# xyang9527/dro-sfm

Measured on AMD Instinct MI355X. Metric: training images/sec (KITTI 192x640 mf self-sup), higher is better.
Workload: dtype f32; 1 GPU; KITTI 192x640 mf self-sup (configs[1]); model=DepthPoseNet it8-seq4-inter-out, global_batch=2, per_gpu_batch=2, ref_frames=2, parallelism=dp1, optimizer=Adam lr 2e-4, execution=hipgraph, update_blocks=depth block + pose block (side stream, with both context encoders), encoder_3x3_s1=hip, encoder_strided=hip, exchange=none (world 1)

## Files before the change

### dro-sfm_amd/csrc/conv.hip

```cpp
#include <hip/hip_runtime.h>

#include <algorithm>
#include <climits>
#include <cstddef>
#include <cstdio>
#include <cstdlib>
#include <cstring>
#include <map>
#include <mutex>
#include <string>
#include <type_traits>

#include "conv_common.hpp"
#include "dro_common.hpp"
#include "wgrad_group_plan.hpp"

namespace dro {


template <int BM, int MODE, int ACT, int EPI>
__global__ __launch_bounds__(256) void igemm_kernel(IgArgs a) {
  constexpr int WM = BM / 32;
  constexpr int KSTEPS = (WM == 2) ? 16 : 8;
  __shared__ float Ws[2][kBK][BM + 1];
// ... 295 lines not shown
}

template <int BM, int KH, int KW, int MODE, int ACT, int EPI, int KS, int XF = 0>
__global__ __launch_bounds__(256 * KS) void dconv_kernel(IgArgs a) {
  using S = HaloShape<BM, KH, KW>;
  {
    const unsigned long long t0 = __builtin_amdgcn_s_memtime();
    if (a.stamps && (threadIdx.x == 0 || threadIdx.x == blockDim.x - 64))
      a.stamps[(size_t)blockIdx.x * 16 + (threadIdx.x == 0 ? 10 : 11)] = t0;
  }
  constexpr int PF = KS <= 2 ? 2 : 1;
  static_assert(KS == 1 || S::LDS >= 4 * 16 * 64, "cross-group reduction area");
  constexpr int T = S::T, TH = S::TH, TW = S::TW, HWd = S::HWd, HALO = S::HALO, HPAD = S::HPAD;
  constexpr int CK = S::CK, NJ = S::NJ, XPER = CK / 4;
  constexpr int RUN = MODE == 0 ? S::RUN0 : S::RUN1, WS = MODE == 0 ? S::WS0 : S::WS1;
  constexpr int WSZ = MODE == 0 ? S::WSZ0 : S::WSZ1, STAGE = S::STAGE;
  constexpr int WM = BM / 32;
  constexpr int PH = KH / 2, PW = KW / 2;
  __shared__ float smem_all[KS * S::LDS];
  const int cb1 = a.cbase[1], cb2 = a.cbase[2], cb3 = a.cbase[3];
  const int H = a.g.H, W = a.g.W;
  const int Cin = a.g.Cin, Cout = a.g.Cout, rows = a.rows, kch = a.kch;
  const int CinT = (MODE == 1 ? a.wcin : Cin) * T;
  const float* __restrict__ Wt = a.weight;
  const float* __restrict__ Gp = a.G;
  const int tid = threadIdx.x & 255, lane = tid & 63;
  const int grp = KS == 1 ? 0 : __builtin_amdgcn_readfirstlane(threadIdx.x >> 8);
  const int wave = __builtin_amdgcn_readfirstlane(tid >> 6);
  float* smem = smem_all + grp * S::LDS;
  const int tile = xcd_remap(blockIdx.x, gridDim.x);
  const int pt = (int)udiv((unsigned)tile, a.rt_div), rt = tile - pt * a.row_tiles;
  const int row0 = rt * BM;
  if constexpr (MODE == 1 && XF == 0 && EPI < 5) {
    const int rl = min(row0 + BM, rows) - 1;
    const int s0 = (row0 >= cb1) + (row0 >= cb2) + (row0 >= cb3);
    const int s1 = (rl >= cb1) + (rl >= cb2) + (rl >= cb3);
    const float* t0 = s0 == 0 ? a.gsrc[0] : s0 == 1 ? a.gsrc[1] : s0 == 2 ? a.gsrc[2] : a.gsrc[3];
    if (s0 == s1 && t0 == nullptr) return;
  }
  const int wcol0 = MODE == 1 ? row0 + (row0 >= a.wgap_at ? a.wgap_len : 0) : row0;
  const int b = (int)udiv((unsigned)pt, a.ti_div), trem = pt - b * a.tiles_img;
  const int tyi = (int)udiv((unsigned)trem, a.tx_div);
  const int ty0 = tyi * TH, tx0 = (trem - tyi * a.tiles_x) * TW;
  const size_t HW = (size_t)H * W;
  const unsigned HWu = (unsigned)HW;
  const int nck = (kch + CK - 1) / CK;
  const int cbeg = blockIdx.y * a.chunks_per_split;
  const int cend = min(nck, cbeg + a.chunks_per_split);

  unsigned xpb[NJ];
  bool xok[NJ], own[NJ];
  static_assert(XF == 0 || ((MODE == 0) == (XF != 3) && ACT == 0), "BN staging transforms: XF 1/2 forward, 3 data gradient");
#pragma unroll
  for (int j = 0; j < NJ; ++j) {
    const int e = lane + 64 * j;
    const int hy = e / HWd, hx = e - hy * HWd;
    const int yy = ty0 - PH + hy, xx = tx0 - PW + hx;
    xok[j] = e < HALO && (unsigned)yy < (unsigned)H && (unsigned)xx < (unsigned)W;
    xpb[j] = xok[j] ? 4u * (unsigned)(yy * W + xx) : 0u;
    own[j] = XF != 0 && xok[j] && hy >= PH && hy < PH + TH && hx >= PW && hx < PW + TW;
  }
  const unsigned wlast = (unsigned)Cout * CinT - 1;

  unsigned long long sQ[4];
  unsigned sR[4], sM[4];
#pragma unroll
  for (int t = 0; t < 4; ++t) {
    if (MODE == 0) {
      sQ[t] = a.sq0[t] + (unsigned long long)b * a.sqb[t];
      sR[t] = a.sr[t];
      sM[t] = a.sm[t];
    } else {
      sQ[t] = reinterpret_cast<unsigned long long>(Gp) + 4ull * (unsigned long long)b * Cout * HW;
      sR[t] = 4u * HWu;
      sM[t] = ~0u;
    }
  }
  const unsigned long long dQ1 = sQ[1] - sQ[0], dQ2 = sQ[2] - sQ[1], dQ3 = sQ[3] - sQ[2];
  const unsigned dR1 = sR[1] - sR[0], dR2 = sR[2] - sR[1], dR3 = sR[3] - sR[2];
  const unsigned dM1 = sM[1] - sM[0], dM2 = sM[2] - sM[1], dM3 = sM[3] - sM[2];
  const long long sbase = MODE == 0 ? reinterpret_cast<long long>(a.src[0].p) : reinterpret_cast<long long>(Gp);
  const long long yshift = reinterpret_cast<long long>(XF == 2 ? a.bn.skip : XF == 3 ? a.bn.z : a.gy) - sbase;
  const long long oshift = reinterpret_cast<long long>(a.bn.yout) - sbase;

  constexpr bool FOLD = MODE == 1 && ACT != 0;
  constexpr bool Y2 = FOLD || XF == 2 || XF == 3;
  constexpr int NXC = XF == 3 ? 5 : 3;
  const float galpha = a.galpha;
  constexpr int W4 = S::WTOT / 4, WPER4 = (W4 + 255) / 256;
  constexpr int WREG = 4 * WPER4;
  static_assert(S::WTOT % 4 == 0 && RUN % 4 == 0, "float4 weight runs");
  unsigned woff[WPER4];
  int wdst[WPER4];
#pragma unroll
  for (int i = 0; i < WPER4; ++i) {
    const int e = 4 * (tid + 256 * i);
    const int run = e / RUN, rem = e - run * RUN;
    woff[i] = (unsigned)run * CinT + (unsigned)rem;
    wdst[i] = (W4 % 256 == 0 || e < S::WTOT) ? run * WS + rem : -1;
  }
  typedef __attribute__((address_space(1))) char* GWPtr;
  struct Stage {
    float xr[XPER * NJ], yr[Y2 ? XPER * NJ : 1], wv[WREG];
    unsigned cmask;
    unsigned ownc;
// ... 274 lines not shown
    }
    if (rowt && !(a.bn.dbg & 2)) bn_put(a.bn.part + (size_t)pt * rows + row, s1, s2);
    if (a.bn.inkernel) bn_finish<EPI>(a, pt, rt, row0, BM);
    stamp(14);
    return;
  }
  for (int e = threadIdx.x; e < BM * 64; e += 256 * KS) {
    const int rl = e >> 6, pl = e & 63;
    float v = 0.f;
#pragma unroll
    for (int g = 0; g < KS; ++g) {
      if (WM == 1)
        v += smem_all[((size_t)(2 * g) * BM + rl) * 64 + pl] + smem_all[((size_t)(2 * g + 1) * BM + rl) * 64 + pl];
      else
        v += smem_all[((size_t)g * BM + rl) * 64 + pl];
    }
    const int row = row0 + rl;
    const int py = pl / TW, px = pl - py * TW;
    const int oy = ty0 + py, ox = tx0 + px;
    if (row >= rows || oy >= H || ox >= W) continue;
    const size_t epix = (size_t)oy * W + ox;
    if (a.part)
      a.part[(size_t)blockIdx.y * rows * P + (size_t)row * P + (size_t)b * HW + epix] = v;
    else
      epi_store<MODE, ACT, EPI>(a, row, b, epix, HW, v);
  }
  stamp(14);
}


__global__ __launch_bounds__(256) void wgrad_kernel(IgArgs a) {
  constexpr int NB = 1;
  __shared__ float Gs[NB][kWP][64 + 1];
  __shared__ float Xs[NB][kWP][64 + 1];
  const int cb1 = a.cbase[1], cb2 = a.cbase[2], cb3 = a.cbase[3];
  const int H = a.g.H, W = a.g.W, KW = a.g.KW, PH = a.g.PH, PW = a.g.PW;
  const int Hsrc = a.Hs, Wsrc = a.Ws, sh = a.sshift;
  const unsigned HWs = (unsigned)Hsrc * (unsigned)Wsrc;
  const int Cin = a.g.Cin, Cout = a.g.Cout;
  const float* __restrict__ Gp = a.G;
  const FastDiv cindiv = a.cindiv, kwdiv = a.kwdiv;
  const int tid = threadIdx.x, lane = tid & 63, wave = tid >> 6;
  const int t = blockIdx.x;
  const int ot = t % a.otiles, nt = t / a.otiles;
  const int o0 = ot * 64, n0 = nt * 64;
  const int NK = a.K;
// ... 1387 lines not shown
      set_error("conv2d: BatchNorm fusion needs a 3x3 stride-1 halo convolution");
      return DRO_E_SHAPE;
    }
    if (EPI >= 5) {
      pl.chunks_per_split = (a.kch + pl.CK - 1) / pl.CK;
      pl.ksplit = 1;
    }
  }
  a.stamps = g_conv_stamps;
  a.dbg = 0;
  if (g_conv_stamps) {
    const char* e = getenv("DRO_CONV_DBG");
    a.dbg = e ? atoi(e) : 0;
  }
  a.K = a.kch * a.g.KH * a.g.KW;
  static const bool thin_off = getenv("DRO_CONV_NO_THIN") != nullptr;
  if (!BNF && !a.flat_only && !thin_off && thin_ok<MODE, EPI>(a)) {
    a.part = reinterpret_cast<float*>(ws);
    return launch_thin<MODE, ACT>(a, pl.ksplit, s);
  }
  if constexpr (EPI < 3 && !BNF) {
    if (!a.flat_only && a.wsplit && xconv_supported(a.g.KH, a.g.KW)) return launch_xconv<MODE, ACT, EPI>(a, ws, s);
  }
  a.row_tiles = pl.row_tiles;
  a.chunks_per_split = pl.chunks_per_split;
  a.part = pl.ksplit > 1 ? reinterpret_cast<float*>(ws) : nullptr;
  const dim3 grid(pl.row_tiles * pl.ptiles, pl.ksplit);
  const double flops = 2.0 * a.rows * a.kch * a.g.KH * a.g.KW * (double)P;
  if (pl.halo)
    conv_logf(flops, "dconv_kernel<%d, %d, %d, %d, %d, %d, %d>", pl.bm, a.g.KH, a.g.KW, MODE, ACT, EPI, pl.kin);
  else
    conv_logf(flops, "igemm_kernel<%d, %d, %d, %d>", pl.bm, MODE, ACT, EPI);
  if (pl.halo) {
    a.TH = pl.TH;
    a.TW = pl.TW;
    a.HWd = pl.HWd;
    a.HPAD = pl.HPAD;
    a.tiles_x = pl.tiles_x;
    a.tiles_img = pl.tiles_img;
    a.CK = pl.CK;
    a.rt_div = make_div32(pl.row_tiles);
    a.ti_div = make_div32(pl.tiles_img);
    a.tx_div = make_div32(pl.tiles_x);
    if (MODE == 0) {
      const unsigned long long HWl = (unsigned long long)a.g.H * a.g.W;
      for (int t = 0; t < kMaxSrc; ++t) {
        const Slice& sl = a.src[t];
        const unsigned long long chs = sl.bcast ? 1ull : HWl;
        const long long cbt = t == 0 ? 0 : a.cbase[t];
        a.sq0[t] = reinterpret_cast<unsigned long long>(sl.p) +
                   4ull * (unsigned long long)(((long long)sl.coff - cbt) * (long long)chs);
        a.sqb[t] = 4ull * (unsigned long long)sl.ctot * chs;
        a.sr[t] = 4u * (unsigned)chs;
        a.sm[t] = sl.bcast ? 0u : ~0u;
      }
    }
    const int KH = a.g.KH;
    const int KW = a.g.KW;
#define DRO_DCONV(BM_, KH_, KW_)                                                                    \
    do {                                                                                            \
      if (pl.kin == 4)                                                                              \
        hipLaunchKernelGGL((dconv_kernel<BM_, KH_, KW_, MODE, ACT, EPI, 4, XF>), grid, dim3(1024), 0, s, a); \
      else if (pl.kin == 2)                                                                         \
        hipLaunchKernelGGL((dconv_kernel<BM_, KH_, KW_, MODE, ACT, EPI, 2, XF>), grid, dim3(512), 0, s, a);  \
// ... 684 lines not shown

extern "C" int dro_conv2d_backward(const dro_slice* srcs, int nsrc, const float* weight, int B, int H,
                                   int W, int Cout, int KH, int KW, int act, float alpha,
                                   const dro_slice* y, const float* dout, float* const* grad_srcs,
                                   const int* grad_ctot, const int* grad_coff,
                                   const int* grad_accumulate, float* grad_weight, float* grad_bias,
                                   int grad_weight_accumulate, const void* wsplit, void* workspace,
                                   size_t workspace_bytes, void* stream) {
  return conv2d_backward_impl(srcs, nsrc, weight, B, H, W, Cout, KH, KW, act, alpha, y, dout, grad_srcs,
                              grad_ctot, grad_coff, grad_accumulate, grad_weight, grad_bias,
                              grad_weight_accumulate, wsplit, workspace, workspace_bytes, stream, nullptr);
}

extern "C" int dro_conv2d_backward_gapped(const dro_slice* srcs, int nsrc, const float* weight, int wcin,
                                          int gap_at, int gap_len, int B, int H, int W, int Cout, int KH,
                                          int KW, const float* dout, float* const* grad_srcs,
                                          const int* grad_ctot, const int* grad_coff,
                                          const int* grad_accumulate, void* workspace, size_t workspace_bytes,
                                          void* stream) {
  const WeightGap gap = {wcin, gap_at, gap_len};
  return conv2d_backward_impl(srcs, nsrc, weight, B, H, W, Cout, KH, KW, 0, 1.f, nullptr, dout, grad_srcs,
                              grad_ctot, grad_coff, grad_accumulate, nullptr, nullptr, 0, nullptr, workspace,
                              workspace_bytes, stream, nullptr, &gap);
}

extern "C" int dro_convgru_candidate_backward(const dro_slice* srcs, int nsrc, const float* weight, int B,
                                              int H, int W, int hd, int KH, int KW, const float* dq,
                                              const float* zr, const float* h, float* dzr, float* dh,
                                              float* const* grad_srcs, const int* grad_ctot,
                                              const int* grad_coff, const int* grad_accumulate,
                                              void* workspace, size_t workspace_bytes, void* stream) {
  if (!srcs || nsrc < 1) {
    set_error("convgru_candidate_backward: need the r*h source");
    return DRO_E_NULL;
  }
  const GruFold gf = {3, zr, h, dzr, dh, nullptr, nullptr, 0};
  return conv2d_backward_impl(srcs, nsrc, weight, B, H, W, hd, KH, KW, 0, 1.f, nullptr, dq, grad_srcs, grad_ctot,
                              grad_coff, grad_accumulate, nullptr, nullptr, 0, nullptr, workspace, workspace_bytes,
                              stream, &gf);
}

extern "C" int dro_convgru_gates_backward(const dro_slice* srcs, int nsrc, const float* weight, int B, int H,
                                          int W, int hd, int KH, int KW, const float* dzr_in,
                                          float* const* grad_srcs, const int* grad_ctot, const int* grad_coff,
                                          const int* grad_accumulate, const float* prev_zr, const float* prev_q,
                                          const float* prev_h, float* prev_dq, float* prev_dzr, float* prev_dh,
// ... 646 lines not shown
```

### dro-sfm_amd/csrc/conv_common.hpp

```cpp
#pragma once
#include <hip/hip_runtime.h>

#include <cstddef>

#include "dro_common.hpp"

namespace dro {

typedef float f32x16 __attribute__((ext_vector_type(16)));

constexpr int kBN = 64;
constexpr int kBK = 32;
constexpr int kWP = 64;
constexpr int kMaxSrc = 4;

struct Slice {
  const float* p;
  int C, ctot, coff;
  int bcast;
};

struct FastDiv {
  unsigned m;
  int one;
// ... 76 lines not shown
  int kch;
  int K;
  FastDiv kdiv, kwdiv, cindiv;
  int row_tiles;
  int chunks_per_split;
  float* part;
  float* bpart;
  int otiles;
  long long pchunk;
  int TH, TW, HWd, HPAD, tiles_x, tiles_img, CK;
  Div32 rt_div, ti_div, tx_div;
  unsigned long long sq0[kMaxSrc], sqb[kMaxSrc];
  unsigned sr[kMaxSrc], sm[kMaxSrc];
  const char* wsplit;
  unsigned long long wplane;
  unsigned wrow;
  int Hs, Ws, sshift;
  int flat_only;
  int pclass;
  long long pcmax;
  unsigned long long* stamps;
  int dbg;
  BnFuse bn;
};

#ifndef DRO_CONV_ABLATE
#define DRO_CONV_ABLATE 0
#endif
__device__ __forceinline__ int ablation_flags(int dbg) { return DRO_CONV_ABLATE ? dbg : 0; }

__device__ __forceinline__ float act_fwd(float v, int act) {
  switch (act) {
    case 1: return fmaxf(v, 0.f);
    case 2: return 1.f / (1.f + expf(-v));
    case 3: return tanhf(v);
    default: return v;
  }
}

__device__ __forceinline__ float act_bwd(float y, int act) {
  switch (act) {
    case 1: return y > 0.f ? 1.f : 0.f;
    case 2: return y * (1.f - y);
    case 3: return 1.f - y * y;
    default: return 1.f;
  }
}
// ... 72 lines not shown
      const size_t i1 = ((size_t)eb * a.hd + row) * HW + epix;
      const float z = a.z.p[zi], qv = a.g1q[i1], hv = a.h.p[((size_t)eb * a.h.ctot + a.h.coff + row) * HW + epix];
      a.g1dq[i1] = gn * z * (1.f - qv * qv);
      a.aux[zi] = gn * (qv - hv) * z * (1.f - z);
      a.g1dh[i1] = a.g1acc ? a.g1dh[i1] + gn * (1.f - z) : gn * (1.f - z);
    } else if (EPI == 3 && row < a.cbase[1]) {
      const size_t zi = ((size_t)eb * a.z.ctot + a.z.coff + row) * HW + epix;
      const size_t hi = ((size_t)eb * a.h.ctot + a.h.coff + row) * HW + epix;
      const float r = a.z.p[zi];
      a.aux[zi] = acc * a.h.p[hi] * r * (1.f - r);
      float* q = a.gsrc[0] + ((size_t)eb * a.gsrc_ctot[0] + a.gsrc_coff[0] + row) * HW + epix;
      *q += acc * r;
    } else if (row < a.cbase[1])
      grad_put(a.gsrc[0], a.gsrc_ctot[0], a.gsrc_coff[0], a.gsrc_acc[0], row, eb, epix, HW, acc);
    else if (row < a.cbase[2])
      grad_put(a.gsrc[1], a.gsrc_ctot[1], a.gsrc_coff[1], a.gsrc_acc[1], row - a.cbase[1], eb, epix, HW, acc);
    else if (row < a.cbase[3])
      grad_put(a.gsrc[2], a.gsrc_ctot[2], a.gsrc_coff[2], a.gsrc_acc[2], row - a.cbase[2], eb, epix, HW, acc);
    else
      grad_put(a.gsrc[3], a.gsrc_ctot[3], a.gsrc_coff[3], a.gsrc_acc[3], row - a.cbase[3], eb, epix, HW, acc);
  }
}

template <int MODE, int ACT, int EPI>
__device__ __forceinline__ void epi_tile(const IgArgs& a, const f32x16& acc, int rbase, int eb,
                                         size_t epix, size_t HW) {
  const int rows = a.rows;
  if (MODE == 0) {
    float bv[16], zv[EPI == 1 ? 16 : 1], hv[EPI != 0 ? 16 : 1];
#pragma unroll
    for (int r = 0; r < 16; ++r) {
      const int row = rbase + (r & 3) + 8 * (r >> 2);
      const int rr = row < rows ? row : 0;
      bv[r] = a.bias ? a.bias[rr] : 0.f;
      if (EPI == 1) {
        zv[r] = a.z.p[((size_t)eb * a.z.ctot + a.z.coff + rr) * HW + epix];
        hv[r] = a.h.p[((size_t)eb * a.h.ctot + a.h.coff + rr) * HW + epix];
      }
      if (EPI == 2) {
        const int c = rr >= a.hd ? rr - a.hd : 0;
        hv[r] = a.h.p[((size_t)eb * a.h.ctot + a.h.coff + c) * HW + epix];
      }
    }
#pragma unroll
    for (int r = 0; r < 16; ++r) {
      const int row = rbase + (r & 3) + 8 * (r >> 2);
// ... 124 lines not shown
```

### dro-sfm_amd/hip/_lib.py

```python
import ctypes
import os

import torch

_HERE = os.path.dirname(os.path.abspath(__file__))
LIB_PATH = os.environ.get("DRO_LIB_PATH") or os.path.normpath(os.path.join(_HERE, "..", "libdro_amd.so"))

_c_float_p = ctypes.c_void_p
_lib = None


def _sig(fn, *argtypes, restype=ctypes.c_int):
    fn.argtypes = list(argtypes)
    fn.restype = restype


def load():
    global _lib
    if _lib is not None:
        return _lib
    if not os.path.exists(LIB_PATH):
        raise RuntimeError(
            f"dro_sfm_amd: native library not found at {LIB_PATH}; build it with "
            "`make -C dro-sfm_amd/csrc` (or __graft_entry__.build()).  There is no CPU fallback.")
# ... 55 lines not shown
    _sig(lib.dro_resize_rgb8_to_tensor, P, I, I, I, I, I, P, P, I, P, P, I, P, P, S)
    _sig(lib.dro_color_jitter_rgb8, P, I, I, I, P, P, S)
    _sig(lib.dro_resize_rgb8, P, I, I, I, I, I, P, P, I, P, P, I, P, P, S)
    _sig(lib.dro_rgb8_to_tensor, P, I, I, I, P, S)
    _sig(lib.dro_png_filtered_bytes, I, I, I, restype=Z)
    _sig(lib.dro_png_decode, P, P, I, I, I, I, P, P, P, S)
    _sig(lib.dro_batchnorm_workspace_bytes, I, I, I, restype=Z)
    _sig(lib.dro_batchnorm_relu_forward, P, P, P, P, I, I, I, I, F, F, P, P, P, P, P, P, P, Z, S)
    _sig(lib.dro_batchnorm_relu_backward, P, P, P, P, P, P, I, I, I, I, P, P, P, P, P, Z, S)
    _sig(lib.dro_conv2d_workspace_bytes, I, I, I, I, I, I, I, restype=Z)
    _sig(lib.dro_conv2d_plan, I, I, I, I, I, I, I, P)
    _sig(lib.dro_conv2d_plan_cin, I, I, I, I, I, I, I, I, P)
    _sig(lib.dro_conv2d_strided_plan, I, I, I, I, I, I, I, I, I, P)
    _sig(lib.dro_debug_conv_stamps, P)
    _sig(lib.dro_conv_log, I)
    _sig(lib.dro_conv_log_read, ctypes.c_char_p, ctypes.c_longlong, restype=ctypes.c_longlong)
    _sig(lib.dro_weight_split_bytes, I, I, I, I, I, restype=Z)
    _sig(lib.dro_weight_split, P, I, I, I, I, P, P, S)
    _sig(lib.dro_conv2d_forward, P, I, P, P, I, I, I, I, I, I, I, F, P, I, I, P, P, Z, S)
    _sig(lib.dro_convgru_gates_forward, P, I, P, P, I, I, I, I, I, I, P, P, P, P, Z, S)
    _sig(lib.dro_convgru_blend_forward, P, I, P, P, I, I, I, I, I, I, P, P, P, P, I, I, P, P, Z, S)
    _sig(lib.dro_conv2d_backward, P, I, P, I, I, I, I, I, I, I, F, P, P, P, P, P, P, P, P, I, P, P, Z, S)
    _sig(lib.dro_conv2d_backward_gapped, P, I, P, I, I, I, I, I, I, I, I, I, P, P, P, P, P, P, Z, S)
    _sig(lib.dro_sum_n, P, I, P, LL, P, I, P, LL, S)
    _sig(lib.dro_conv2d_weight_grad_multi_workspace_bytes, I, I, I, I, I, I, I, I, restype=Z)
    _sig(lib.dro_conv2d_weight_grad_multi, P, I, I, I, I, I, I, I, I, I, F, P, P, I, P, Z, S)
    _sig(lib.dro_conv2d_weight_grad_group_capacity, P, P)
    _sig(lib.dro_conv2d_weight_grad_group_workspace_bytes, P, I, I, I, restype=Z)
    _sig(lib.dro_conv2d_weight_grad_group, P, I, I, I, I, P, Z, S)
    _sig(lib.dro_conv2d_weight_grad_multi_ex, P, I, I, I, I, I, I, I, I, I, F, P, P, I, P, P, Z, S)
    _sig(lib.dro_conv2d_weight_grad_group_ex, P, P, I, I, I, I, P, Z, S)
    _sig(lib.dro_adam_step, P, P, P, P, ctypes.c_longlong, P, P, S)
    _sig(lib.dro_gru_backward_elem, I, I, I, I, I, P, P, P, P, P, P, P, P, S)
    _sig(lib.dro_convgru_candidate_backward, P, I, P, I, I, I, I, I, I, P, P, P, P, P, P, P, P, P, P, Z, S)
    _sig(lib.dro_convgru_gates_backward, P, I, P, I, I, I, I, I, I, P, P, P, P, P, P, P, P, P, P, P, I, P, Z, S)
    _sig(lib.dro_bn_state_bytes, I, I, I, I, restype=Z)
    _sig(lib.dro_bn_apply, P, P, I, I, I, I, I, P, P, S)
    _sig(lib.dro_bn_backward_apply, P, P, I, I, I, I, P, P, S)
    _sig(lib.dro_conv2d_bn_forward, P, I, I, I, I, P, I, P, P, P, P, P, P, P, Z, S)
    _sig(lib.dro_conv2d_bn_backward_data, P, I, I, I, I, I, P, P, P, P, P, P, P, I, P, Z, S)
    _lib = lib
    return lib


EXPORTED = (
    "dro_last_error", "dro_abi_version", "dro_timestamp", "dro_wall_clock_hz",
    "dro_warp_cost_forward", "dro_warp_cost_workspace_bytes", "dro_warp_cost_backward",
    "dro_view_synthesis_forward", "dro_view_synthesis_backward",
    "dro_plane_sweep_forward",
    "dro_photometric_workspace_bytes", "dro_photometric_clip_offset", "dro_photometric_forward", "dro_photometric_backward",
    "dro_supervised_workspace_bytes", "dro_supervised_forward", "dro_supervised_backward",
    "dro_convex_upsample_forward", "dro_convex_upsample_backward",
    "dro_convex_upsample_many_forward", "dro_convex_upsample_many_workspace_bytes",
    "dro_convex_upsample_many_backward",
    "dro_bilinear_upsample2x_forward", "dro_bilinear_upsample2x_backward",
    "dro_maxpool3x3s2_forward", "dro_maxpool3x3s2_backward",
    "dro_depth_metrics_blocks", "dro_depth_metrics_workspace_bytes", "dro_depth_metrics_prepare",
    "dro_depth_metrics_reduce", "dro_depth_metrics_median_workspace_bytes", "dro_depth_metrics_median",
    "dro_depth_metrics_demon_prepare", "dro_depth_metrics_demon_reduce", "dro_post_process_inv_depth",
    "dro_depth_clean", "dro_depth_fusion", "dro_backproject_points_workspace_bytes", "dro_backproject_points",
    "dro_render_points_workspace_bytes", "dro_render_points",
    "dro_conv2d_strided_workspace_bytes", "dro_conv2d_strided_forward", "dro_conv2d_strided_backward",
    "dro_pose_mean_forward", "dro_pose_mean_backward",
    "dro_resize_rgb8_to_tensor", "dro_color_jitter_rgb8", "dro_resize_rgb8", "dro_rgb8_to_tensor",
    "dro_png_filtered_bytes", "dro_png_decode",
    "dro_batchnorm_workspace_bytes", "dro_batchnorm_relu_forward", "dro_batchnorm_relu_backward",
    "dro_weight_split_bytes", "dro_weight_split",
    "dro_conv2d_workspace_bytes", "dro_conv2d_plan", "dro_conv2d_plan_cin", "dro_conv2d_strided_plan", "dro_debug_conv_stamps", "dro_conv_log", "dro_conv_log_read", "dro_conv2d_forward", "dro_convgru_gates_forward",
    "dro_convgru_blend_forward", "dro_conv2d_backward", "dro_conv2d_backward_gapped", "dro_sum_n",
    "dro_conv2d_weight_grad_multi_workspace_bytes", "dro_conv2d_weight_grad_multi",
    "dro_conv2d_weight_grad_group_capacity", "dro_conv2d_weight_grad_group_workspace_bytes",
    "dro_conv2d_weight_grad_group", "dro_conv2d_weight_grad_multi_ex", "dro_conv2d_weight_grad_group_ex",
    "dro_gru_backward_elem", "dro_convgru_candidate_backward", "dro_convgru_gates_backward", "dro_adam_step",
    "dro_bn_state_bytes", "dro_bn_apply", "dro_bn_backward_apply", "dro_conv2d_bn_forward", "dro_conv2d_bn_backward_data",
    "dro_percentile", "dro_colorize", "dro_depth_png16_rows",
)


def check(status, what):
    if status != 0:
        msg = load().dro_last_error().decode(errors="replace")
        raise RuntimeError(f"{what} failed (status {status}): {msg}")


def ptr(t):
    return ctypes.c_void_p(t.data_ptr()) if t is not None else ctypes.c_void_p(0)


def stream_of(t):
    return ctypes.c_void_p(torch.cuda.current_stream(t.device).cuda_stream)


# ... 10 lines not shown
```

### dro-sfm_amd/hip/conv.py

```python
import contextlib
import ctypes
import os
from typing import Optional

import torch

from . import _lib
from ._lib import check, ptr, require_device, stream_of
from .ops import _sink_of

ACT = {None: 0, "none": 0, "relu": 1, "sigmoid": 2, "tanh": 3}


class DroSlice(ctypes.Structure):
    _fields_ = [("data", ctypes.c_void_p), ("channels", ctypes.c_int),
                ("total_channels", ctypes.c_int), ("channel_offset", ctypes.c_int),
                ("broadcast", ctypes.c_int)]


def _slice(t):
    B, C, H, W = t.shape
    s0, s1, s2, s3 = t.stride()
    if s2 == 0 and s3 == 0 and s1 == 1:
        return DroSlice(t.data_ptr(), C, s0 if B > 1 else C, 0, 1)
# ... 503 lines not shown
    rw = gw if (first and need_w) else None
    rb = gb if (first and has_bias and need_b) else None
    return gsrc, rw, rb, None, None, none_params, None


torch.library.register_autograd("dro::conv2d", _conv2d_backward, setup_context=_conv2d_setup)


def conv2d(srcs, weight, bias=None, act=None, alpha=1.0, parts=None):
    if torch.is_tensor(srcs):
        srcs = [srcs]
    if parts is None:
        parts = ((weight,), (bias,) if bias is not None else ())
    wparts, bparts = parts
    direct = _direct_targets(wparts, bparts)
    if direct is not None:
        return torch.ops.dro.conv2d(list(srcs), direct[0], direct[1], ACT[act], float(alpha),
                                    [*wparts, *bparts], len(wparts))
    if weight is None:
        key = ("cat",) + tuple(id(p) for p in wparts)
        weight, bias = cached_cat(key, lambda: (torch.cat(list(wparts), 0),
                                                torch.cat(list(bparts), 0) if bparts else None))
    return torch.ops.dro.conv2d(list(srcs), weight, bias, ACT[act], float(alpha), [], 0)


@torch.library.custom_op("dro::conv2d_strided", mutates_args=())
def _conv2d_strided_op(x: Tensor, weight: Tensor, bias: Optional[Tensor], stride: int, pad: int,
                       act: int) -> Tensor:
    lib = _lib.load()
    require_device(x, weight, bias, what="conv2d_strided")
    B, Cin, Hi, Wi = x.shape
    Cout, cin_w, KH, KW = weight.shape
    if cin_w != Cin:
        raise RuntimeError("conv2d_strided: input channels do not match the weight")
    Ho, Wo = (Hi + 2 * pad - KH) // stride + 1, (Wi + 2 * pad - KW) // stride + 1
    x, weight = x.contiguous(), weight.contiguous()
    out = torch.empty(B, Cout, Ho, Wo, device=x.device, dtype=torch.float32)
    nws = int(lib.dro_conv2d_strided_workspace_bytes(B, Hi, Wi, Cin, Cout, KH, KW, stride, pad))
    ws = torch.empty(max(nws, 1), dtype=torch.uint8, device=x.device)
    check(lib.dro_conv2d_strided_forward(ptr(x), ptr(weight), ptr(bias), B, Hi, Wi, Cin, Cout, KH, KW, stride, pad,
                                         act, ptr(out), ptr(ws), nws, stream_of(out)), "dro_conv2d_strided_forward")
    return out


@_conv2d_strided_op.register_fake
def _(x, weight, bias, stride, pad, act):
# ... 498 lines not shown
```

### dro-sfm_amd/networks/optim/update.py

```python
import torch
import torch.nn as nn
import torch.nn.functional as F

from ... import hip
from ...hip import conv as hip_conv

_BACKEND = "hip"
_ACT_FN = {None: lambda x: x, "relu": F.relu, "sigmoid": torch.sigmoid, "tanh": torch.tanh}


def set_conv_backend(name):
    global _BACKEND
    if name not in ("hip", "miopen"):
        raise ValueError(name)
    _BACKEND = name


def conv_backend():
    return _BACKEND


def declare(module, table):
    for name, (cin, cout, k, pad) in table.items():
        setattr(module, name, nn.Conv2d(cin, cout, k, padding=pad))
# ... 80 lines not shown
        q = conv([r * h, *xs], cq.weight, cq.bias, "tanh")
        return (1 - z) * h + z * q

    def dro_param_groups(self):
        return fused_groups(self.convz1, self.convr1) + fused_groups(self.convz2, self.convr2)

    def forward(self, h, x, context=None):
        xs = _as_list(x)
        chain = hip_conv.GruChain() if _BACKEND == "hip" else None
        return self._gate(self._gate(h, xs, "1", chain, context), xs, "2", chain, context)


class _Projection(nn.Module):

    def __init__(self, tag, state_ch, cost_dim, hidden_dim, out_chs):
        super().__init__()
        self.out_chs, self._tag = out_chs, tag
        declare(self, {"convc1": (cost_dim, hidden_dim, 1, 0),
                       "convc2": (hidden_dim, hidden_dim, 3, 1),
                       f"conv{tag}1": (state_ch, hidden_dim, 7, 3),
                       f"conv{tag}2": (hidden_dim, 64, 3, 1),
                       f"conv{tag}": (64 + hidden_dim, out_chs - state_ch, 3, 1)})

    def sources(self, state_map, cost):
        t = self._tag
        c1, c2 = self.convc1, self.convc2
        s1, s2, f = (getattr(self, f"conv{t}{i}") for i in ("1", "2", ""))
        cor = relu_rec(conv(relu_rec(conv(cost, c1.weight, c1.bias, "relu"), c1), c2.weight, c2.bias, "relu"), c2)
        sfm = relu_rec(conv(relu_rec(conv(state_map, s1.weight, s1.bias, "relu"), s1), s2.weight, s2.bias, "relu"),
                       s2)
        return [hip.grad_sink(relu_rec(conv([cor, sfm], f.weight, f.bias, "relu"), f)), state_map]


class ProjectionInputDepth(_Projection):
    def __init__(self, cost_dim, hidden_dim, out_chs):
        super().__init__("d", 1, cost_dim, hidden_dim, out_chs)

    def forward(self, depth, cost):
        return torch.cat(self.sources(depth, cost), 1)


class ProjectionInputPose(_Projection):
    def __init__(self, cost_dim, hidden_dim, out_chs):
        super().__init__("p", 6, cost_dim, hidden_dim, out_chs)

    def pose_map(self, pose, cost):
        bs, _, h, w = cost.shape
        return pose.reshape(bs, 6, 1, 1).expand(bs, 6, h, w)

    def sources(self, pose, cost):
# ... 65 lines not shown
```

### include/dro_amd.h

```cpp
#ifndef DRO_AMD_H
#define DRO_AMD_H

#include <stddef.h>

#ifdef __cplusplus
extern "C" {
#endif

#define DRO_POSE_EULER 0
#define DRO_POSE_MATRIX 1

#define DRO_DEPTH_METRIC 0
#define DRO_DEPTH_INV 1
#define DRO_DEPTH_DISP 2

#define DRO_OK 0
#define DRO_E_NULL (-1)
#define DRO_E_SHAPE (-2)
#define DRO_E_MODE (-3)

const char* dro_last_error(void);
int dro_abi_version(void);

int dro_timestamp(unsigned long long* buf, int slot, void* stream);
// ... 213 lines not shown
                              const float* bias, int B, int H, int W, int hd, int KH, int KW,
                              float* zr, float* rh, const void* wsplit, void* workspace,
                              size_t workspace_bytes, void* stream);

int dro_convgru_blend_forward(const dro_slice* srcs, int nsrc, const float* weight,
                              const float* bias, int B, int H, int W, int Cout, int KH, int KW,
                              const dro_slice* z, const dro_slice* h, float* q_out, float* out,
                              int out_ctot, int out_coff, const void* wsplit, void* workspace,
                              size_t workspace_bytes, void* stream);

int dro_conv2d_backward(const dro_slice* srcs, int nsrc, const float* weight, int B, int H, int W,
                        int Cout, int KH, int KW, int act, float alpha, const dro_slice* y,
                        const float* dout, float* const* grad_srcs, const int* grad_ctot,
                        const int* grad_coff, const int* grad_accumulate, float* grad_weight,
                        float* grad_bias, int grad_weight_accumulate, const void* wsplit,
                        void* workspace, size_t workspace_bytes, void* stream);

int dro_conv2d_backward_gapped(const dro_slice* srcs, int nsrc, const float* weight, int wcin, int gap_at,
                               int gap_len, int B, int H, int W, int Cout, int KH, int KW,
                               const float* dout, float* const* grad_srcs, const int* grad_ctot,
                               const int* grad_coff, const int* grad_accumulate, void* workspace,
                               size_t workspace_bytes, void* stream);

int dro_sum_n(const float* const* srcs_a, int na, float* out_a, long long numel_a,
              const float* const* srcs_b, int nb, float* out_b, long long numel_b, void* stream);

size_t dro_conv2d_strided_workspace_bytes(int B, int Hi, int Wi, int Cin, int Cout, int KH, int KW,
                                          int stride, int pad);
int dro_conv2d_strided_forward(const float* x, const float* weight, const float* bias, int B, int Hi,
                               int Wi, int Cin, int Cout, int KH, int KW, int stride, int pad, int act,
                               float* out, void* workspace, size_t workspace_bytes, void* stream);
int dro_conv2d_strided_backward(const float* x, const float* weight, const float* dout, int B, int Hi,
                                int Wi, int Cin, int Cout, int KH, int KW, int stride, int pad,
                                float* grad_x, int grad_x_accumulate, float* grad_weight,
                                float* grad_bias, int grad_weight_accumulate, void* workspace,
                                size_t workspace_bytes, void* stream);

int dro_pose_mean_forward(const float* y, const float* pose, float* out, int B, int C, int HW,
                          float rot_scale, void* stream);
int dro_pose_mean_backward(const float* gout, float* gy, int B, int C, int HW, float rot_scale,
                           void* stream);

typedef struct dro_wgrad_use {
  const dro_slice* srcs;
  const float* dout;
  const float* y;
// ... 108 lines not shown
```

Baseline: 144.9 images/s.

## Batch the cost and state second 3x3 convs into one paired launch

Adds a paired conv kernel mode in which one grid covers two independent same-shape 3x3 convolutions. Blocks in the second half of the row-tile range shift their source, weight, bias and output pointers by precomputed byte deltas. The motion encoder's convc2 and conv*2 layers, plus their data-gradient backward, now run as one launch each instead of two, aiming to cut launch count and fill more of the GPU with small convs. The cost is a mask computation and pointer arithmetic per block, restricted to halo 32-row plans without split-K, with a fallback to two launches otherwise.

```diff
diff --git a/dro-sfm_amd/csrc/conv.hip b/dro-sfm_amd/csrc/conv.hip
--- a/dro-sfm_amd/csrc/conv.hip
+++ b/dro-sfm_amd/csrc/conv.hip
@@ -341,15 +341,19 @@
   const int H = a.g.H, W = a.g.W;
   const int Cin = a.g.Cin, Cout = a.g.Cout, rows = a.rows, kch = a.kch;
   const int CinT = (MODE == 1 ? a.wcin : Cin) * T;
-  const float* __restrict__ Wt = a.weight;
-  const float* __restrict__ Gp = a.G;
   const int tid = threadIdx.x & 255, lane = tid & 63;
   const int grp = KS == 1 ? 0 : __builtin_amdgcn_readfirstlane(threadIdx.x >> 8);
   const int wave = __builtin_amdgcn_readfirstlane(tid >> 6);
   float* smem = smem_all + grp * S::LDS;
   const int tile = xcd_remap(blockIdx.x, gridDim.x);
-  const int pt = (int)udiv((unsigned)tile, a.rt_div), rt = tile - pt * a.row_tiles;
+  const int pt = (int)udiv((unsigned)tile, a.rt_div), rt_all = tile - pt * a.row_tiles;
+  constexpr bool PAIRED = EPI == 0 && XF == 0 && KH == 3 && KW == 3 && BM == 32;
+  const int prt = PAIRED ? a.pair_row_tiles : 0;
+  const long long pm = PAIRED ? pair_mask(rt_all, prt) : 0LL;
+  const int rt = rt_all - ((int)pm & prt);
   const int row0 = rt * BM;
+  const float* __restrict__ Wt = PAIRED ? pair_shift(a.weight, a.pair_dweight, pm) : a.weight;
+  const float* __restrict__ Gp = PAIRED ? pair_shift(a.G, a.pair_dG, pm) : a.G;
   if constexpr (MODE == 1 && XF == 0 && EPI < 5) {
     const int rl = min(row0 + BM, rows) - 1;
     const int s0 = (row0 >= cb1) + (row0 >= cb2) + (row0 >= cb3);
@@ -387,6 +391,7 @@
   for (int t = 0; t < 4; ++t) {
     if (MODE == 0) {
       sQ[t] = a.sq0[t] + (unsigned long long)b * a.sqb[t];
+      if (PAIRED) sQ[t] += (unsigned long long)(a.pair_dsrc & pm);
       sR[t] = a.sr[t];
       sM[t] = a.sm[t];
     } else {
@@ -399,7 +404,8 @@
   const unsigned dR1 = sR[1] - sR[0], dR2 = sR[2] - sR[1], dR3 = sR[3] - sR[2];
   const unsigned dM1 = sM[1] - sM[0], dM2 = sM[2] - sM[1], dM3 = sM[3] - sM[2];
   const long long sbase = MODE == 0 ? reinterpret_cast<long long>(a.src[0].p) : reinterpret_cast<long long>(Gp);
-  const long long yshift = reinterpret_cast<long long>(XF == 2 ? a.bn.skip : XF == 3 ? a.bn.z : a.gy) - sbase;
+  const long long yshift = reinterpret_cast<long long>(XF == 2 ? a.bn.skip : XF == 3 ? a.bn.z : a.gy) - sbase +
+                           (PAIRED ? a.pair_dgy & pm : 0LL);
   const long long oshift = reinterpret_cast<long long>(a.bn.yout) - sbase;
 
   constexpr bool FOLD = MODE == 1 && ACT != 0;
@@ -720,6 +726,8 @@
     const size_t epix = (size_t)oy * W + ox;
     if (a.part)
       a.part[(size_t)blockIdx.y * rows * P + (size_t)row * P + (size_t)b * HW + epix] = v;
+    else if constexpr (PAIRED)
+      epi_store_pair<MODE, ACT>(a, pm, row, b, epix, HW, v);
     else
       epi_store<MODE, ACT, EPI>(a, row, b, epix, HW, v);
   }
@@ -2153,11 +2161,18 @@
   if constexpr (EPI < 3 && !BNF) {
     if (!a.flat_only && a.wsplit && xconv_supported(a.g.KH, a.g.KW)) return launch_xconv<MODE, ACT, EPI>(a, ws, s);
   }
-  a.row_tiles = pl.row_tiles;
+  const bool pair = a.pair_row_tiles != 0;
+  if (pair && (EPI != 0 || XF != 0 || !pl.halo || pl.ksplit != 1 || pl.bm != 32 || a.g.KH != 3 || a.g.KW != 3)) {
+    set_error("conv2d_pair: needs a 3x3 halo-kernel conv with 32-row tiles, the plain epilogue and no split-K over blocks");
+    return DRO_E_SHAPE;
+  }
+  const int grid_rt = pair ? 2 * pl.row_tiles : pl.row_tiles;
+  a.pair_row_tiles = pair ? pl.row_tiles : 0;
+  a.row_tiles = grid_rt;
   a.chunks_per_split = pl.chunks_per_split;
   a.part = pl.ksplit > 1 ? reinterpret_cast<float*>(ws) : nullptr;
-  const dim3 grid(pl.row_tiles * pl.ptiles, pl.ksplit);
-  const double flops = 2.0 * a.rows * a.kch * a.g.KH * a.g.KW * (double)P;
+  const dim3 grid(grid_rt * pl.ptiles, pl.ksplit);
+  const double flops = (pair ? 4.0 : 2.0) * a.rows * a.kch * a.g.KH * a.g.KW * (double)P;
   if (pl.halo)
     conv_logf(flops, "dconv_kernel<%d, %d, %d, %d, %d, %d, %d>", pl.bm, a.g.KH, a.g.KW, MODE, ACT, EPI, pl.kin);
   else
@@ -2170,7 +2185,7 @@
     a.tiles_x = pl.tiles_x;
     a.tiles_img = pl.tiles_img;
     a.CK = pl.CK;
-    a.rt_div = make_div32(pl.row_tiles);
+    a.rt_div = make_div32(grid_rt);
     a.ti_div = make_div32(pl.tiles_img);
     a.tx_div = make_div32(pl.tiles_x);
     if (MODE == 0) {
@@ -2901,6 +2916,152 @@
   return conv2d_backward_impl(srcs, nsrc, weight, B, H, W, Cout, KH, KW, 0, 1.f, nullptr, dout, grad_srcs,
                               grad_ctot, grad_coff, grad_accumulate, nullptr, nullptr, 0, nullptr, workspace,
                               workspace_bytes, stream, nullptr, &gap);
+}
+
+static bool pair_plan(int rows, int kch, int KH, int KW, int B, int H, int W, int cin, IgPlan* out) {
+  const IgPlan pl = plan_igemm(rows, kch, KH, KW, B, H, W, cin);
+  if (out) *out = pl;
+  return pl.halo && KH == 3 && KW == 3 && pl.bm == 32 && pl.ksplit == 1 &&
+         2LL * pl.row_tiles * pl.ptiles < (1LL << 30);
+}
+
+extern "C" int dro_conv2d_pair_plan(int rows, int kch, int KH, int KW, int B, int H, int W, int cin, int epi,
+                                    int xf, long long* info, int* supported) {
+  if (!info || !supported) {
+    set_error("conv2d_pair_plan: NULL info/supported");
+    return DRO_E_NULL;
+  }
+  *supported = 0;
+  if (rows < 1 || kch < 1 || KH < 1 || KW < 1 || B < 1 || H < 1 || W < 1 || cin < 0) {
+    set_error("conv2d_pair_plan: bad arguments");
+    return DRO_E_SHAPE;
+  }
+  if (epi != 0 || xf != 0) {
+    set_error("conv2d_pair_plan: only the plain epilogue (EPI 0) and untransformed staging (XF 0) pair");
+    return DRO_E_MODE;
+  }
+  IgPlan pl;
+  *supported = pair_plan(rows, kch, KH, KW, B, H, W, cin, &pl) ? 1 : 0;
+  const long long v[16] = {pl.halo, pl.bm, pl.row_tiles, pl.ptiles, pl.ksplit, pl.chunks_per_split,
+                           pl.TH, pl.TW, pl.HWd, pl.HPAD, pl.tiles_x, pl.tiles_img, pl.CK,
+                           (long long)pl.lds_bytes, (long long)pl.part_bytes, pl.kin};
+  for (int i = 0; i < 16; ++i) info[i] = v[i];
+  return DRO_OK;
+}
+
+static long long byte_delta(const void* second, const void* first) {
+  return (long long)(reinterpret_cast<intptr_t>(second) - reinterpret_cast<intptr_t>(first));
+}
+
+static int pair_setup(IgArgs& a, const char* what, const dro_slice* src_a, const dro_slice* src_b, int B, int H,
+                      int W, int Cout, int KH, int KW, int act, float alpha, int epi, int xf) {
+  static thread_local char msg[160];
+  if (!src_a || !src_b || !src_a->data || !src_b->data) {
+    snprintf(msg, sizeof(msg), "%s: NULL source", what);
+    set_error(msg);
+    return DRO_E_NULL;
+  }
+  if (epi != 0 || xf != 0) {
+    snprintf(msg, sizeof(msg), "%s: only the plain epilogue (EPI 0) and untransformed staging (XF 0) pair", what);
+    set_error(msg);
+    return DRO_E_MODE;
+  }
+  if (act < 0 || act > 3 || (alpha != 1.f && act != 0)) {
+    snprintf(msg, sizeof(msg), "%s: unknown activation, or alpha != 1 with one", what);
+    set_error(msg);
+    return DRO_E_MODE;
+  }
+  if (src_a->channels != src_b->channels || src_a->total_channels != src_b->total_channels || src_a->broadcast ||
+      src_b->broadcast) {
+    snprintf(msg, sizeof(msg), "%s: the members need dense sources of equal channels", what);
+    set_error(msg);
+    return DRO_E_SHAPE;
+  }
+  int st = conv_setup_geom(a, src_a, 1, B, H, W, Cout, KH, KW);
+  if (st) return st;
+  dro_slice sb = *src_b;
+  IgArgs b = {};
+  if ((st = conv_setup_geom(b, &sb, 1, B, H, W, Cout, KH, KW))) return st;
+  return DRO_OK;
+}
+
+extern "C" int dro_conv2d_pair(const dro_slice* src_a, const dro_slice* src_b, const float* weight_a,
+                               const float* weight_b, const float* bias_a, const float* bias_b, int B, int H,
+                               int W, int Cout, int KH, int KW, int act, float alpha, int epi, int xf,
+                               float* out_a, float* out_b, void* stream) {
+  IgArgs a = {};
+  int st = pair_setup(a, "conv2d_pair", src_a, src_b, B, H, W, Cout, KH, KW, act, alpha, epi, xf);
+  if (st) return st;
+  if (!weight_a || !weight_b || !out_a || !out_b || (bias_a == nullptr) != (bias_b == nullptr)) {
+    set_error("conv2d_pair: NULL weight/out, or a bias in one member only");
+    return DRO_E_NULL;
+  }
+  if (!pair_plan(Cout, a.g.Cin, KH, KW, B, H, W, a.g.Cin, nullptr)) {
+    set_error("conv2d_pair: unsupported (needs the halo kernel without split-K over blocks: "
+              "dro_conv2d_pair_plan); run the members as two launches");
+    return DRO_E_SHAPE;
+  }
+  const long long HW4 = 4LL * H * W;
+  a.weight = weight_a;
+  a.bias = bias_a;
+  a.alpha = alpha;
+  a.out = out_a;
+  a.out_ctot = Cout;
+  a.out_coff = 0;
+  a.rows = Cout;
+  a.kch = a.g.Cin;
+  a.pair_row_tiles = 1;
+  a.pair_dsrc = byte_delta(src_b->data, src_a->data) + HW4 * (src_b->channel_offset - src_a->channel_offset);
+  a.pair_dweight = byte_delta(weight_b, weight_a);
+  a.pair_dbias = bias_a ? byte_delta(bias_b, bias_a) : 0;
+  a.pair_dout = byte_delta(out_b, out_a);
+  const long long P = (long long)B * H * W;
+  hipStream_t s = (hipStream_t)stream;
+  DRO_ACT_SWITCH(act, st = (launch_igemm<0, A_, 0>(a, P, nullptr, s)));
+  return st;
+}
+
+extern "C" int dro_conv2d_pair_backward(const float* weight_a, const float* weight_b, int B, int H, int W,
+                                        int Cin, int Cout, int KH, int KW, int act, float alpha, int epi, int xf,
+                                        const float* y_a, const float* y_b, const float* dout_a,
+                                        const float* dout_b, float* grad_a, float* grad_b, int grad_ctot,
+                                        int grad_coff, int grad_accumulate, void* stream) {
+  if (!weight_a || !weight_b || !dout_a || !dout_b || !grad_a || !grad_b || (act != 0 && (!y_a || !y_b))) {
+    set_error("conv2d_pair_backward: NULL weight/dout/grad/y");
+    return DRO_E_NULL;
+  }
+  if (Cin < 1 || grad_coff < 0 || grad_coff + Cin > grad_ctot || too_big(B, grad_ctot, (long long)H * W)) {
+    set_error("conv2d_pair_backward: bad gradient target slice");
+    return DRO_E_SHAPE;
+  }
+  const dro_slice sa = {dout_a, Cin, Cin, 0, 0}, sb = {dout_b, Cin, Cin, 0, 0};
+  IgArgs a = {};
+  int st = pair_setup(a, "conv2d_pair_backward", &sa, &sb, B, H, W, Cout, KH, KW, act, alpha, epi, xf);
+  if (st) return st;
+  if (!pair_plan(Cin, Cout, KH, KW, B, H, W, Cin, nullptr)) {
+    set_error("conv2d_pair_backward: unsupported (needs the halo kernel without split-K over blocks: "
+              "dro_conv2d_pair_plan); run the members as two launches");
+    return DRO_E_SHAPE;
+  }
+  a.weight = weight_a;
+  a.G = dout_a;
+  a.galpha = alpha;
+  a.gy = act ? y_a : nullptr;
+  a.gsrc[0] = grad_a;
+  a.gsrc_ctot[0] = grad_ctot;
+  a.gsrc_coff[0] = grad_coff;
+  a.gsrc_acc[0] = grad_accumulate ? 1 : 0;
+  a.rows = Cin;
+  a.kch = Cout;
+  a.pair_row_tiles = 1;
+  a.pair_dweight = byte_delta(weight_b, weight_a);
+  a.pair_dG = byte_delta(dout_b, dout_a);
+  a.pair_dgy = act ? byte_delta(y_b, y_a) : 0;
+  a.pair_dgsrc = byte_delta(grad_b, grad_a);
+  const long long P = (long long)B * H * W;
+  hipStream_t s = (hipStream_t)stream;
+  DRO_ACT_SWITCH(act, st = (launch_igemm<1, A_, 0>(a, P, nullptr, s)));
+  return st;
 }
 
 extern "C" int dro_convgru_candidate_backward(const dro_slice* srcs, int nsrc, const float* weight, int B,
diff --git a/dro-sfm_amd/csrc/conv_common.hpp b/dro-sfm_amd/csrc/conv_common.hpp
--- a/dro-sfm_amd/csrc/conv_common.hpp
+++ b/dro-sfm_amd/csrc/conv_common.hpp
@@ -122,7 +122,20 @@
   unsigned long long* stamps;
   int dbg;
   BnFuse bn;
-};
+  int pair_row_tiles;
+  long long pair_dsrc;
+  long long pair_dweight, pair_dbias, pair_dout;
+  long long pair_dG, pair_dgy;
+  long long pair_dgsrc;
+};
+
+__device__ __forceinline__ long long pair_mask(int rt, int pair_row_tiles) {
+  return (unsigned)(rt - pair_row_tiles) < (unsigned)pair_row_tiles ? -1LL : 0LL;
+}
+template <typename T>
+__device__ __forceinline__ T* pair_shift(T* p, long long delta, long long mask) {
+  return reinterpret_cast<T*>(reinterpret_cast<long long>(p) + (delta & mask));
+}
 
 #ifndef DRO_CONV_ABLATE
 #define DRO_CONV_ABLATE 0
@@ -241,6 +254,21 @@
   }
 }
 
+template <int MODE, int ACT>
+__device__ __forceinline__ void epi_store_pair(const IgArgs& a, long long pm, int row, int eb, size_t epix,
+                                               size_t HW, float acc) {
+  if (MODE == 0) {
+    float v = acc + (a.bias ? pair_shift(a.bias, a.pair_dbias, pm)[row] : 0.f);
+    v = a.alpha * act_fwd(v, ACT);
+    pair_shift(a.out, a.pair_dout, pm)[((size_t)eb * a.out_ctot + a.out_coff + row) * HW + epix] = v;
+  } else if (row < a.cbase[1]) {
+    grad_put(a.gsrc[0] ? pair_shift(a.gsrc[0], a.pair_dgsrc, pm) : nullptr, a.gsrc_ctot[0], a.gsrc_coff[0],
+             a.gsrc_acc[0], row, eb, epix, HW, acc);
+  } else {
+    epi_store<MODE, ACT, 0>(a, row, eb, epix, HW, acc);
+  }
+}
+
 template <int MODE, int ACT, int EPI>
 __device__ __forceinline__ void epi_tile(const IgArgs& a, const f32x16& acc, int rbase, int eb,
                                          size_t epix, size_t HW) {
diff --git a/dro-sfm_amd/hip/_lib.py b/dro-sfm_amd/hip/_lib.py
--- a/dro-sfm_amd/hip/_lib.py
+++ b/dro-sfm_amd/hip/_lib.py
@@ -101,6 +101,9 @@
     _sig(lib.dro_convgru_blend_forward, P, I, P, P, I, I, I, I, I, I, P, P, P, P, I, I, P, P, Z, S)
     _sig(lib.dro_conv2d_backward, P, I, P, I, I, I, I, I, I, I, F, P, P, P, P, P, P, P, P, I, P, P, Z, S)
     _sig(lib.dro_conv2d_backward_gapped, P, I, P, I, I, I, I, I, I, I, I, I, P, P, P, P, P, P, Z, S)
+    _sig(lib.dro_conv2d_pair_plan, I, I, I, I, I, I, I, I, I, I, P, P)
+    _sig(lib.dro_conv2d_pair, P, P, P, P, P, P, I, I, I, I, I, I, I, F, I, I, P, P, S)
+    _sig(lib.dro_conv2d_pair_backward, P, P, I, I, I, I, I, I, I, I, F, I, I, P, P, P, P, P, P, I, I, I, S)
     _sig(lib.dro_sum_n, P, I, P, LL, P, I, P, LL, S)
     _sig(lib.dro_conv2d_weight_grad_multi_workspace_bytes, I, I, I, I, I, I, I, I, restype=Z)
     _sig(lib.dro_conv2d_weight_grad_multi, P, I, I, I, I, I, I, I, I, I, F, P, P, I, P, Z, S)
@@ -147,6 +150,7 @@
     "dro_weight_split_bytes", "dro_weight_split",
     "dro_conv2d_workspace_bytes", "dro_conv2d_plan", "dro_conv2d_plan_cin", "dro_conv2d_strided_plan", "dro_debug_conv_stamps", "dro_conv_log", "dro_conv_log_read", "dro_conv2d_forward", "dro_convgru_gates_forward",
     "dro_convgru_blend_forward", "dro_conv2d_backward", "dro_conv2d_backward_gapped", "dro_sum_n",
+    "dro_conv2d_pair_plan", "dro_conv2d_pair", "dro_conv2d_pair_backward",
     "dro_conv2d_weight_grad_multi_workspace_bytes", "dro_conv2d_weight_grad_multi",
     "dro_conv2d_weight_grad_group_capacity", "dro_conv2d_weight_grad_group_workspace_bytes",
     "dro_conv2d_weight_grad_group", "dro_conv2d_weight_grad_multi_ex", "dro_conv2d_weight_grad_group_ex",
diff --git a/dro-sfm_amd/hip/conv.py b/dro-sfm_amd/hip/conv.py
--- a/dro-sfm_amd/hip/conv.py
+++ b/dro-sfm_amd/hip/conv.py
@@ -549,6 +549,157 @@
         weight, bias = cached_cat(key, lambda: (torch.cat(list(wparts), 0),
                                                 torch.cat(list(bparts), 0) if bparts else None))
     return torch.ops.dro.conv2d(list(srcs), weight, bias, ACT[act], float(alpha), [], 0)
+
+
+_PAIRS = [os.environ.get("DRO_CONV_PAIR", "1") != "0"]
+_PAIR_PLANS = {}
+
+
+def set_conv_pairs(enabled):
+    _PAIRS[0] = bool(enabled)
+
+
+def conv_pairs():
+    return _PAIRS[0]
+
+
+def _pair_plan_ok(rows, kch, KH, KW, B, H, W, cin):
+    key = (rows, kch, KH, KW, B, H, W, cin)
+    v = _PAIR_PLANS.get(key)
+    if v is None:
+        info, sup = (ctypes.c_longlong * 16)(), ctypes.c_int(0)
+        check(_lib.load().dro_conv2d_pair_plan(rows, kch, KH, KW, B, H, W, cin, 0, 0, info, ctypes.byref(sup)),
+              "dro_conv2d_pair_plan")
+        v = _PAIR_PLANS[key] = bool(sup.value)
+    return v
+
+
+def conv_pair_supported(shape_a, shape_b, wshape_a, wshape_b):
+    if tuple(shape_a) != tuple(shape_b) or tuple(wshape_a) != tuple(wshape_b) or len(shape_a) != 4:
+        return False
+    B, C, H, W = shape_a
+    Cout, Cin, KH, KW = wshape_a
+    if C != Cin or _XCONV[0]:
+        return False
+    return _pair_plan_ok(Cout, Cin, KH, KW, B, H, W, Cin) and _pair_plan_ok(Cin, Cout, KH, KW, B, H, W, Cin)
+
+
+def _pair_dense(t):
+    return t.is_cuda and t.dtype == torch.float32 and t.dim() == 4 and t.is_contiguous()
+
+
+@torch.library.custom_op("dro::conv2d_pair", mutates_args=())
+def _conv2d_pair_op(xa: Tensor, xb: Tensor, wa: Tensor, wb: Tensor, ba: Optional[Tensor], bb: Optional[Tensor],
+                    act: int, alpha: float, params: list[Tensor], nweight: int) -> tuple[Tensor, Tensor]:
+    lib = _lib.load()
+    require_device(xa, xb, wa, wb, ba, bb, what="conv2d_pair")
+    Cout, Cin, KH, KW = wa.shape
+    B, _, H, W = xa.shape
+    wa, wb = wa.contiguous(), wb.contiguous()
+    ya, yb = _dense_out([xa], Cout), _dense_out([xb], Cout)
+    sa, sb = _slice(xa), _slice(xb)
+    check(lib.dro_conv2d_pair(ctypes.byref(sa), ctypes.byref(sb), ptr(wa), ptr(wb), ptr(ba), ptr(bb), B, H, W,
+                              Cout, KH, KW, act, ctypes.c_float(alpha), 0, 0, ptr(ya), ptr(yb), stream_of(ya)),
+          "dro_conv2d_pair")
+    return ya, yb
+
+
+@_conv2d_pair_op.register_fake
+def _(xa, xb, wa, wb, ba, bb, act, alpha, params, nweight):
+    B, _, H, W = xa.shape
+    return xa.new_empty((B, wa.shape[0], H, W)), xb.new_empty((B, wb.shape[0], H, W))
+
+
+def _conv2d_pair_setup(ctx, inputs, output):
+    xa, xb, wa, wb, ba, bb, act, alpha, params, nweight = inputs
+    ya, yb = output
+    ctx.save_for_backward(wa.contiguous(), wb.contiguous(), ya if act else None, yb if act else None, xa, xb)
+    ctx.sinks = [_sink_of(x) if x.requires_grad else None for x in (xa, xb)]
+    ctx.need_src = [x.requires_grad for x in (xa, xb)]
+    has_bias = ba is not None
+    ctx.meta = (act, alpha, has_bias, (wa.requires_grad, wb.requires_grad),
+                (has_bias and ba.requires_grad, has_bias and bb.requires_grad))
+    ctx.direct = None
+    if params:
+        bias = params[nweight:]
+        ctx.direct = [_direct_targets((params[i],), (bias[i],) if bias else (), mark=False, in_setup=True)
+                      for i in range(2)]
+    ctx.scope = None if params else current_scope()
+    ctx.nparams = len(params)
+
+
+def _pair_data_grads(ws, ys, gouts, act, alpha, tgt, dacc):
+    Cout, Cin, KH, KW = ws[0].shape
+    B, _, H, W = gouts[0].shape
+    check(_lib.load().dro_conv2d_pair_backward(
+        ptr(ws[0]), ptr(ws[1]), B, H, W, Cin, Cout, KH, KW, act, ctypes.c_float(alpha), 0, 0, ptr(ys[0]), ptr(ys[1]),
+        ptr(gouts[0]), ptr(gouts[1]), ptr(tgt[0]), ptr(tgt[1]), Cin, 0, int(dacc[0]), stream_of(gouts[0])),
+        "dro_conv2d_pair_backward")
+
+
+def _conv2d_pair_backward(ctx, ga, gb_):
+    wa, wb, ya, yb, xa, xb = ctx.saved_tensors
+    act, alpha, has_bias, need_w, need_b = ctx.meta
+    ws, ys, xs = (wa, wb), (ya, yb), (xa, xb)
+    Cout, Cin, KH, KW = wa.shape
+    B, _, H, W = xa.shape
+    gouts = [g.contiguous() for g in (ga, gb_)]
+    dev = gouts[0].device
+    sinks = ctx.sinks
+    gsrc = [torch.empty(B, Cin, H, W, device=dev) if ctx.need_src[i] and sinks[i] is None else None
+            for i in range(2)]
+    sk = [sn.target() if sn is not None else (None, 0) for sn in sinks]
+    tgt = [t if sn is not None else g for (t, _), sn, g in zip(sk, sinks, gsrc)]
+    dacc = [a for _, a in sk]
+    if (tgt[0] is not None and tgt[1] is not None and dacc[0] == dacc[1] and _pair_dense(tgt[0])
+            and _pair_dense(tgt[1])):
+        _pair_data_grads(ws, ys, gouts, act, alpha, tgt, dacc)
+    else:
+        for i in range(2):
+            if tgt[i] is not None:
+                _conv_bwd([xs[i]], ws[i], ys[i], gouts[i], act, alpha, [tgt[i]], [dacc[i]])
+    none_params = [None] * ctx.nparams
+    rw, rb = [None, None], [None, None]
+    for i in (1, 0):
+        if ctx.direct is not None:
+            gw, gb = ctx.direct[i][2], ctx.direct[i][3] if has_bias else None
+            if not _queue_weight_grad([xs[i]], ws[i].shape, act, alpha, gouts[i], ys[i], gw, gb, ws[i]):
+                _conv_bwd([xs[i]], ws[i], ys[i], gouts[i], act, alpha, [None], [0], gw, gb, 1)
+        elif need_w[i] or need_b[i]:
+            gw, gb, wacc, first = _grad_buffers(ctx.scope, ("conv", ws[i].data_ptr(), Cout), ws[i],
+                                                Cout if has_bias else 0, dev)
+            _conv_bwd([xs[i]], ws[i], ys[i], gouts[i], act, alpha, [None], [0], gw, gb, wacc)
+            rw[i] = gw if (first and need_w[i]) else None
+            rb[i] = gb if (first and need_b[i]) else None
+    return gsrc[0], gsrc[1], rw[0], rw[1], rb[0], rb[1], None, None, none_params, None
+
+
+torch.library.register_autograd("dro::conv2d_pair", _conv2d_pair_backward, setup_context=_conv2d_pair_setup)
+
+
+def conv2d_pair(srcs_a, srcs_b, conv_a, conv_b, act=None, alpha=1.0):
+    srcs_a = [srcs_a] if torch.is_tensor(srcs_a) else list(srcs_a)
+    srcs_b = [srcs_b] if torch.is_tensor(srcs_b) else list(srcs_b)
+    (wa, ba), (wb, bb) = conv_a, conv_b
+
+    def two():
+        return conv2d(srcs_a, wa, ba, act, alpha), conv2d(srcs_b, wb, bb, act, alpha)
+
+    if not (_PAIRS[0] and len(srcs_a) == 1 and len(srcs_b) == 1 and (ba is None) == (bb is None)
+            and _pair_dense(srcs_a[0]) and _pair_dense(srcs_b[0])
+            and conv_pair_supported(srcs_a[0].shape, srcs_b[0].shape, wa.shape, wb.shape)):
+        return two()
+    xa, xb = srcs_a[0], srcs_b[0]
+    bparts = ((ba,), (bb,)) if ba is not None else ((), ())
+    direct = [_direct_targets((w,), bp, mark=False) for w, bp in zip((wa, wb), bparts)]
+    if direct[0] is not None and direct[1] is not None:
+        _mark_direct([wa, wb, *bparts[0], *bparts[1]])
+        (w0, b0, _, _), (w1, b1, _, _) = direct
+        return torch.ops.dro.conv2d_pair(xa, xb, w0, w1, b0, b1, ACT[act], float(alpha),
+                                         [wa, wb, *bparts[0], *bparts[1]], 2)
+    if direct[0] is not None or direct[1] is not None:
+        return two()
+    return torch.ops.dro.conv2d_pair(xa, xb, wa, wb, ba, bb, ACT[act], float(alpha), [], 0)
 
 
 @torch.library.custom_op("dro::conv2d_strided", mutates_args=())
diff --git a/dro-sfm_amd/networks/optim/update.py b/dro-sfm_amd/networks/optim/update.py
--- a/dro-sfm_amd/networks/optim/update.py
+++ b/dro-sfm_amd/networks/optim/update.py
@@ -126,10 +126,24 @@
                        f"conv{tag}2": (hidden_dim, 64, 3, 1),
                        f"conv{tag}": (64 + hidden_dim, out_chs - state_ch, 3, 1)})
 
+    def _pairs(self, cost, c2, s2):
+        if _BACKEND != "hip" or not cost.is_cuda or not hip_conv.conv_pairs():
+            return False
+        B, _, H, W = cost.shape
+        shape = (B, c2.in_channels, H, W)
+        return (c2.weight.shape == s2.weight.shape
+                and hip_conv.conv_pair_supported(shape, shape, c2.weight.shape, s2.weight.shape))
+
     def sources(self, state_map, cost):
         t = self._tag
         c1, c2 = self.convc1, self.convc2
         s1, s2, f = (getattr(self, f"conv{t}{i}") for i in ("1", "2", ""))
+        if self._pairs(cost, c2, s2):
+            a = relu_rec(conv(cost, c1.weight, c1.bias, "relu"), c1)
+            b = conv(state_map, s1.weight, s1.bias, "relu")
+            cor, sfm = hip_conv.conv2d_pair(a, b, (c2.weight, c2.bias), (s2.weight, s2.bias), "relu")
+            cor, b, sfm = relu_rec(cor, c2), relu_rec(b, s1), relu_rec(sfm, s2)
+            return [hip.grad_sink(relu_rec(conv([cor, sfm], f.weight, f.bias, "relu"), f)), state_map]
         cor = relu_rec(conv(relu_rec(conv(cost, c1.weight, c1.bias, "relu"), c1), c2.weight, c2.bias, "relu"), c2)
         sfm = relu_rec(conv(relu_rec(conv(state_map, s1.weight, s1.bias, "relu"), s1), s2.weight, s2.bias, "relu"),
                        s2)
diff --git a/include/dro_amd.h b/include/dro_amd.h
--- a/include/dro_amd.h
+++ b/include/dro_amd.h
@@ -259,6 +259,18 @@
                                const int* grad_coff, const int* grad_accumulate, void* workspace,
                                size_t workspace_bytes, void* stream);
 
+int dro_conv2d_pair_plan(int rows, int kch, int KH, int KW, int B, int H, int W, int cin, int epi, int xf,
+                         long long* info, int* supported);
+int dro_conv2d_pair(const dro_slice* src_a, const dro_slice* src_b, const float* weight_a,
+                    const float* weight_b, const float* bias_a, const float* bias_b, int B, int H, int W,
+                    int Cout, int KH, int KW, int act, float alpha, int epi, int xf, float* out_a,
+                    float* out_b, void* stream);
+int dro_conv2d_pair_backward(const float* weight_a, const float* weight_b, int B, int H, int W, int Cin,
+                             int Cout, int KH, int KW, int act, float alpha, int epi, int xf,
+                             const float* y_a, const float* y_b, const float* dout_a, const float* dout_b,
+                             float* grad_a, float* grad_b, int grad_ctot, int grad_coff, int grad_accumulate,
+                             void* stream);
+
 int dro_sum_n(const float* const* srcs_a, int na, float* out_a, long long numel_a,
               const float* const* srcs_b, int nb, float* out_b, long long numel_b, void* stream);
 
```

After: 141.1 images/s. 0.974x the previous value.
